# refresh-bio/DSRC

Measured on AMD Instinct MI355X. Metric: raw FASTQ MB/s compressed (bit-identical .dsrc) at -d3 -q2, higher is better.
Workload: dtype u8/u16/u32 integer

## Files before the change

### dsrc_amd/csrc/dsrc_gpu.hip

```cpp
#include <hip/hip_runtime.h>

#include <algorithm>
#include <atomic>
#include <cstdarg>
#include <cstdio>
#include <cstdlib>
#include <cstring>
#include <chrono>
#include <condition_variable>
#include <deque>
#include <functional>
#include <dlfcn.h>
#include <mutex>
#ifndef DSRC_REPLAY_WHATIF
#define DSRC_REPLAY_WHATIF 0
#endif
#include <string>
#include <thread>
#include <vector>

#include "../../include/dsrc_gpu.h"
#include "dsrc_types.h"
#include "k_common.h"
#ifndef RCS_WIDE
// ... 729 lines not shown
	HIPCHK(hipMemcpyAsync(d_desc, desc.data(), sizeof(BlkDesc) * B, hipMemcpyHostToDevice, s));
	HIPCHK(hipMemcpyAsync(d_tplan, tplan.data(), sizeof(TagPlan) * B, hipMemcpyHostToDevice, s));
	HIPCHK(hipMemcpyAsync(d_tres, tres.data(), sizeof(TagFieldRes) * tres.size(), hipMemcpyHostToDevice, s));
	hipLaunchKernelGGL(k_tag_hist, dim3(B), dim3(WG), 0, s, d_in, d_desc, d_state, rp, wpool, wpool, d_tplan, d_tres); KCHK();
	hipLaunchKernelGGL(k_tag_trees, dim3((DSRC_MAX_FIELDS * DSRC_MAX_STRF + 63) / 64, B), dim3(64), 0, s, d_state, wpool, d_tplan, d_tres); KCHK();
	hipLaunchKernelGGL(k_tag_emit, dim3(B), dim3(WG), 0, s, d_in, d_desc, d_state, rp, wpool, spool, wpool, wpool, d_tplan, d_tres); KCHK();
	hipLaunchKernelGGL(k_tag_raw, dim3(B), dim3(WG), 0, s, d_in, d_desc, d_state, rp, wpool, wpool, d_tplan); KCHK();

	if (zero_hi > zero_lo) HIPCHK(hipMemsetAsync(h->arena.base + zero_lo, 0, zero_hi - zero_lo, s));
	HIPCHK(hipMemcpyAsync(d_desc, desc.data(), sizeof(BlkDesc) * B, hipMemcpyHostToDevice, s));
	HIPCHK(hipMemcpyAsync(d_qplan, qplan.data(), sizeof(QuaPlan) * B, hipMemcpyHostToDevice, s));
	HIPCHK(hipMemcpyAsync(d_dplan, dplan.data(), sizeof(QuaPlan) * B, hipMemcpyHostToDevice, s));
	if (NJ)
	{
		HIPCHK(hipMemcpyAsync(d_jobs, jobs.data(), sizeof(CtxJob) * NJ, hipMemcpyHostToDevice, s));
		HIPCHK(hipMemcpyAsync(d_chains, chains.data(), sizeof(RcChain) * NJ, hipMemcpyHostToDevice, s));
	}

	u32 maxq = 1, maxd = 1, max_len = 1, max_qn = 1;
	for (u32 b = 0; b < B; ++b) { maxq = std::max(maxq, st[b].q_total); maxd = std::max(maxd, st[b].d_total); max_len = std::max(max_len, st[b].max_len); max_qn = std::max(max_qn, st[b].q_count); }

	if (qo == 0)
	{
		hipLaunchKernelGGL(k_qpos_hist, dim3(B), dim3(WG), 0, s, d_desc, d_state, rp, d_q, wpool, d_qplan); KCHK();
		hipLaunchKernelGGL(k_qpos_trees, dim3((max_len + 63) / 64, B), dim3(64), 0, s, d_state, wpool, d_qplan); KCHK();
		hipLaunchKernelGGL(k_qpos_emit, dim3(B), dim3(WG), 0, s, d_desc, d_state, rp, d_q, wpool, wpool, d_qplan); KCHK();
		hipLaunchKernelGGL(k_qrle_runs, dim3(B), dim3(WG), 0, s, d_desc, d_state, d_q, wpool, d_qplan); KCHK();
		hipLaunchKernelGGL(k_qrle_hist, dim3(B), dim3(WG), 0, s, d_desc, d_state, d_q, wpool, d_qplan); KCHK();
		hipLaunchKernelGGL(k_qrle_trees, dim3((2 * max_qn + 63) / 64, B), dim3(64), 0, s, d_state, wpool, d_qplan); KCHK();
		hipLaunchKernelGGL(k_qrle_emit, dim3(B), dim3(WG), 0, s, d_desc, d_state, d_q, wpool, wpool, d_qplan); KCHK();
	}
	if (dna_order == 0)
	{
		const u32 gx = std::max(1u, std::min(64u, (maxd / 4 + WG - 1) / WG));
		hipLaunchKernelGGL(k_dna_b2, dim3(gx, B), dim3(WG), 0, s, d_desc, d_state, d_d, wpool); KCHK();
		hipLaunchKernelGGL(k_dna_huff, dim3(B), dim3(WG), 0, s, d_desc, d_state, d_d, wpool, wpool, d_dplan); KCHK();
	}
	hipLaunchKernelGGL(k_dna_none, dim3((B + 63) / 64), dim3(64), 0, s, d_desc, d_state, wpool, B); KCHK();
	h->rc_launches = 0;
	std::function<int(const BkGroup&)> launch_fallback;
	u32* d_bk = use_bk ? AP<u32>(h, o_bk) : nullptr;
	u32* d_redo = AP<u32>(h, o_redo);
	const bool rc_one_lane = hook_env("DSRC_GPU_RC_ONE_LANE") != nullptr;
	if (NJ)
	{
		const u32 nq = (u32)qjobs.size(), nd = (u32)djobs.size();
		const bool sort_atomic = h->sort_atomic;
		hipLaunchKernelGGL(k_rc_headers, dim3((NJ + 63) / 64), dim3(64), 0, s, d_jobs, NJ, d_state, wpool); KCHK();
		HIPCHK(hipMemsetAsync(d_redo, 0, ((size_t)NJ + 2) * 4, s));
		u16* d_bcnt = use_bk ? AP<u16>(h, o_bcnt) : nullptr;
		if (use_bk) HIPCHK(hipMemsetAsync(d_bk, 0, bk_zero_words * 4, s));
		const u32 max_parts = 2048u;
		launch_fallback = [&, sort_atomic, max_parts](const BkGroup& g) -> int
		{
			const u32 cnt = g.hi - g.lo;
			const u32* fb = d_bk + g.fb;
			if (sort_atomic) hipLaunchKernelGGL((k_sort<0, true>), dim3(std::min(cnt, 16u)), dim3(SORT_WG), 0, s, d_jobs, lpool, d_d, d_q, d_qp, d_state, fb);
			else hipLaunchKernelGGL((k_sort<0, false>), dim3(std::min(cnt, 16u)), dim3(SORT_WG), 0, s, d_jobs, lpool, d_d, d_q, d_qp, d_state, fb);
			u32 mxn = 1; for (u32 i = g.lo; i < g.hi; ++i) mxn = std::max(mxn, jobs[i].n);
			const u32 parts = std::max(1u, std::min(max_parts, mxn / 1024u));
			const dim3 rgrid(parts * std::min(cnt, 4u));
#define BK_REPLAY(NN) { hipLaunchKernelGGL(k_replay_seams<NN>, rgrid, dim3(REPLAY_WG), 0, s, d_jobs, const_cast<u64*>(lpool), parts, cnt, fb); \
					hipLaunchKernelGGL((k_replay<NN, 0>), rgrid, dim3(REPLAY_WG), 0, s, d_jobs, lpool, AP<RcPack>(h, 0), parts, cnt, fb); }
			switch (jobs[g.lo].n_alpha)
			{
			case 4: BK_REPLAY(4) break; case 8: BK_REPLAY(8) break; case 16: BK_REPLAY(16) break;
			case 32: BK_REPLAY(32) break; case 64: BK_REPLAY(64) break; default: BK_REPLAY(128) break;
			}
#undef BK_REPLAY
			KCHK();
			return 0;
		};
		for (size_t sl = 0; sl + 1 < slice_lo.size(); ++sl)
		{
			const u32 s_lo = slice_lo[sl], s_hi = slice_lo[sl + 1];
			stage_mark(0);
			if (use_bk)
			{
				u32 slice_bins = 0;
				for (u32 i = s_lo; i < s_hi; ++i) if (jobs[i].bk_on) slice_bins = std::max(slice_bins, (jobs[i].n + BK_BIN - 1) >> BK_TB);
				hipLaunchKernelGGL(k_part, dim3(std::max(1u, slice_bins), s_hi - s_lo), dim3(PART_WG), 0, s, d_jobs + s_lo, lpool, d_d, d_q, d_qp, d_state, d_bk, d_bcnt);
				KCHK();
				stage_mark(0); stage_mark(1);
				if (slice_bins) { hipLaunchKernelGGL(k_binoff, dim3(slice_bins, s_hi - s_lo), dim3(256), 0, s, d_jobs + s_lo, d_bcnt, d_bk); KCHK(); }
				for (const BkGroup& g : bk_groups[sl])
				{
					u32 hb = 0; bool any = false;
					for (u32 i = g.lo; i < g.hi; ++i) if (jobs[i].bk_on) { any = true; hb = std::max(hb, jobs[i].bk_hb); }
					if (!any) continue;
					u32 lbm = 0; for (u32 i = g.lo; i < g.hi; ++i) if (jobs[i].bk_on) lbm = std::max(lbm, jobs[i].bk_lb);
#define BK_LAUNCH(NN, MB, RB) hipLaunchKernelGGL((k_model<NN, MB, RB>), dim3(((1u << hb) + MD_WAVES_FOR(RB) - 1) / MD_WAVES_FOR(RB), g.hi - g.lo), dim3(64 * MD_WAVES_FOR(RB)), 0, s, d_jobs + g.lo, lpool, AP<RcPack>(h, 0), d_bk, d_bcnt, (RcPack*)(d_bk + ((bk_zero_words + 1) & ~(size_t)1)))
#define BK_FINISH(NN) { if ((1u << lbm) * 4 * MdRow<NN>::STRIDE <= 4096) BK_LAUNCH(NN, 0, 4096); \
						else if ((1u << lbm) * 4 * MdRow<NN>::STRIDE <= MD_ROW_BYTES) BK_LAUNCH(NN, 0, MD_ROW_BYTES); \
						else if (lbm <= 10) BK_LAUNCH(NN, 10, MD_ROW_BYTES); \
						else BK_LAUNCH(NN, BK_MAX_LB, MD_ROW_BYTES); }
					switch (jobs[g.lo].n_alpha)
					{
					case 4: BK_FINISH(4) break; case 8: BK_FINISH(8) break; case 16: BK_FINISH(16) break;
					case 32: BK_FINISH(32) break; case 64: BK_FINISH(64) break; default: BK_FINISH(128) break;
					}
#undef BK_LAUNCH
#undef BK_FINISH
					KCHK();
				}
				if (bk_binned && slice_bins) { hipLaunchKernelGGL(k_place, dim3(slice_bins, s_hi - s_lo), dim3(PLACE_WG), 0, s, d_jobs + s_lo, lpool, AP<RcPack>(h, 0), d_bk); KCHK(); }
				for (const BkGroup& g : bk_groups[sl])
				{
					bool known = false;
					for (u32 i = g.lo; i < g.hi; ++i) known = known || !jobs[i].bk_on;
					if (known) { const int rc = launch_fallback(g); if (rc) return rc; }
				}
				stage_mark(1);
				continue;
			}
#ifdef DSRC_SORT_PROBE
			{
				static int shots = 0;
				if (sl == 0 && shots < 2)
				{
					++shots;
					hipEvent_t e0, e1; hipEventCreate(&e0); hipEventCreate(&e1);
#define PROBE_RUN(M) { hipEventRecord(e0, s); if (sort_atomic) hipLaunchKernelGGL((k_sort<M, true>), dim3(s_hi - s_lo), dim3(SORT_WG), 0, s, d_jobs + s_lo, lpool, d_d, d_q, d_qp, d_state, nullptr); else hipLaunchKernelGGL((k_sort<M, false>), dim3(s_hi - s_lo), dim3(SORT_WG), 0, s, d_jobs + s_lo, lpool, d_d, d_q, d_qp, d_state, nullptr); \
					hipEventRecord(e1, s); hipEventSynchronize(e1); float ms = 0; hipEventElapsedTime(&ms, e0, e1); fprintf(stderr, "[probe] k_sort<%u> %u streams: %.2f ms\n", (unsigned)M, s_hi - s_lo, ms); }
					PROBE_RUN(0) PROBE_RUN(0) PROBE_RUN(128) PROBE_RUN(129) PROBE_RUN(130) PROBE_RUN(132) PROBE_RUN(134) PROBE_RUN(136) PROBE_RUN(144) PROBE_RUN(160) PROBE_RUN(192) PROBE_RUN(255)
					hipEventDestroy(e0); hipEventDestroy(e1);
				}
			}
#endif
			if (sort_atomic) hipLaunchKernelGGL((k_sort<0, true>), dim3(s_hi - s_lo), dim3(SORT_WG), 0, s, d_jobs + s_lo, lpool, d_d, d_q, d_qp, d_state, nullptr);
			else hipLaunchKernelGGL((k_sort<0, false>), dim3(s_hi - s_lo), dim3(SORT_WG), 0, s, d_jobs + s_lo, lpool, d_d, d_q, d_qp, d_state, nullptr);
			KCHK();
			stage_mark(0); stage_mark(1);
			for (u32 lo = s_lo; lo < s_hi;)
			{
				u32 hi = lo;
				while (hi < s_hi && jobs[hi].n_alpha == jobs[lo].n_alpha) ++hi;
				const u32 cnt = hi - lo;
				u32 mxn = 1; for (u32 i = lo; i < hi; ++i) mxn = std::max(mxn, jobs[i].n);
				const u32 parts = std::max(1u, std::min(max_parts, mxn / 1024u));
				const dim3 rgrid(parts * cnt);
#ifdef DSRC_SORT_PROBE
				{
					static int shots = 0;
					if ((jobs[lo].n_alpha == 32 || jobs[lo].n_alpha == 4) && lo == s_lo && shots < 4 && (sl == 0 || sl + 2 == slice_lo.size()))
					{
						++shots;
						hipEvent_t e0, e1; hipEventCreate(&e0); hipEventCreate(&e1);
#define RPROBE_RUN(NN, M) { hipEventRecord(e0, s); hipLaunchKernelGGL((k_replay<NN, M>), rgrid, dim3(REPLAY_WG), 0, s, d_jobs + lo, lpool, AP<RcPack>(h, 0), parts, cnt, nullptr); \
						hipEventRecord(e1, s); hipEventSynchronize(e1); float ms = 0; hipEventElapsedTime(&ms, e0, e1); fprintf(stderr, "[probe] k_replay<%d,%d> %u streams x %u parts: %.2f ms\n", NN, M, cnt, parts, ms); }
						hipLaunchKernelGGL(k_replay_seams<32>, rgrid, dim3(REPLAY_WG), 0, s, d_jobs + lo, const_cast<u64*>(lpool), parts, cnt, nullptr);
						if (jobs[lo].n_alpha == 32) { RPROBE_RUN(32, 0) RPROBE_RUN(32, 0) RPROBE_RUN(32, 1) RPROBE_RUN(32, 2) RPROBE_RUN(32, 8) RPROBE_RUN(32, 16) }
						else { RPROBE_RUN(4, 0) RPROBE_RUN(4, 0) RPROBE_RUN(4, 1) RPROBE_RUN(4, 2) RPROBE_RUN(4, 8) RPROBE_RUN(4, 16) }
						hipEventDestroy(e0); hipEventDestroy(e1);
					}
				}
#endif
				switch (jobs[lo].n_alpha)
				{
				case 4:   hipLaunchKernelGGL(k_replay_seams<4>, rgrid, dim3(REPLAY_WG), 0, s, d_jobs + lo, const_cast<u64*>(lpool), parts, cnt, nullptr); hipLaunchKernelGGL((k_replay<4, DSRC_REPLAY_WHATIF>), rgrid, dim3(REPLAY_WG), 0, s, d_jobs + lo, lpool, AP<RcPack>(h, 0), parts, cnt, nullptr); break;
				case 8:   hipLaunchKernelGGL(k_replay_seams<8>, rgrid, dim3(REPLAY_WG), 0, s, d_jobs + lo, const_cast<u64*>(lpool), parts, cnt, nullptr); hipLaunchKernelGGL((k_replay<8, DSRC_REPLAY_WHATIF>), rgrid, dim3(REPLAY_WG), 0, s, d_jobs + lo, lpool, AP<RcPack>(h, 0), parts, cnt, nullptr); break;
				case 16:  hipLaunchKernelGGL(k_replay_seams<16>, rgrid, dim3(REPLAY_WG), 0, s, d_jobs + lo, const_cast<u64*>(lpool), parts, cnt, nullptr); hipLaunchKernelGGL((k_replay<16, DSRC_REPLAY_WHATIF>), rgrid, dim3(REPLAY_WG), 0, s, d_jobs + lo, lpool, AP<RcPack>(h, 0), parts, cnt, nullptr); break;
				case 32:  hipLaunchKernelGGL(k_replay_seams<32>, rgrid, dim3(REPLAY_WG), 0, s, d_jobs + lo, const_cast<u64*>(lpool), parts, cnt, nullptr); hipLaunchKernelGGL((k_replay<32, DSRC_REPLAY_WHATIF>), rgrid, dim3(REPLAY_WG), 0, s, d_jobs + lo, lpool, AP<RcPack>(h, 0), parts, cnt, nullptr); break;
				case 64:  hipLaunchKernelGGL(k_replay_seams<64>, rgrid, dim3(REPLAY_WG), 0, s, d_jobs + lo, const_cast<u64*>(lpool), parts, cnt, nullptr); hipLaunchKernelGGL((k_replay<64, DSRC_REPLAY_WHATIF>), rgrid, dim3(REPLAY_WG), 0, s, d_jobs + lo, lpool, AP<RcPack>(h, 0), parts, cnt, nullptr); break;
				default:  hipLaunchKernelGGL(k_replay_seams<128>, rgrid, dim3(REPLAY_WG), 0, s, d_jobs + lo, const_cast<u64*>(lpool), parts, cnt, nullptr); hipLaunchKernelGGL((k_replay<128, DSRC_REPLAY_WHATIF>), rgrid, dim3(REPLAY_WG), 0, s, d_jobs + lo, lpool, AP<RcPack>(h, 0), parts, cnt, nullptr); break;
				}
				KCHK();
				lo = hi;
			}
			stage_mark(1);
		}
		HIPCHK(hipEventRecord(h->ev[4], s));
		HIPCHK(hipStreamWaitEvent(h->rc_stream, h->ev[4], 0));
		HIPCHK(hipEventRecord(h->ev[2], h->rc_stream));
		if (rc_one_lane) hipLaunchKernelGGL(k_rc, dim3((NJ + RC_LANES - 1) / RC_LANES), dim3(64 * RC_WG_WAVES), 0, h->rc_stream, d_chains, NJ, (const u32*)nullptr, AP<RcPack>(h, 0), wpool, d_state);
		else if (NJ > (u32)hook_int("DSRC_GPU_RC_WIDE_FROM", 640)) hipLaunchKernelGGL(k_rcs<RCS_WIDE>, dim3((NJ + RCS_WIDE - 1) / RCS_WIDE), dim3(64 * RCS_WG_WAVES), 0, h->rc_stream, d_chains, NJ, AP<RcPack>(h, 0), wpool, d_state, (const u32*)d_bk, d_redo);
		else hipLaunchKernelGGL(k_rcs<16>, dim3((NJ + 15) / 16), dim3(64 * RCS_WG_WAVES), 0, h->rc_stream, d_chains, NJ, AP<RcPack>(h, 0), wpool, d_state, (const u32*)d_bk, d_redo);
		KCHK();
		HIPCHK(hipEventRecord(h->ev[3], h->rc_stream));
		HIPCHK(hipEventSynchronize(h->ev[3]));
		h->rc_launches = 1;
	}

	hipLaunchKernelGGL(k_meta_plan, dim3((B + 63) / 64), dim3(64), 0, s, d_state, prm); KCHK();

// ... 1426 lines not shown
```

### dsrc_amd/csrc/k_bucket.h

```cpp
#pragma once
#include <type_traits>
#include "k_rc.h"

#define BK_MAX_HB 10
#define BK_MAX_LB 11
#define BK_LIMIT 524288
#define BK_BIG 16384
#ifndef BK_TB
#define BK_TB 13
#endif
#define BK_BIN (1u << BK_TB)
static_assert(BK_TB == RC6_TB, "a time bin is the unit of k_rc's record layout (rc6_chunk_off)");
#ifndef BK_MAX_BINS
#define BK_MAX_BINS 512
#endif
#define BK_MAX_BINS_WIDE 65536
#define BK_HASH_MUL 0x9E3779B1u


__device__ __forceinline__ u64 bk_rekey(const CtxJob& j, u64 el)
{
	const u32 key = ((u32)(el >> ELEM_CTX_SHIFT) * j.bk_mul) & j.bk_kmask;
	return (el & ((1ull << ELEM_CTX_SHIFT) - 1ull)) | ((u64)key << ELEM_CTX_SHIFT);
}
// ... 81 lines not shown
	constexpr u32 tile_elems = PART_WG * PART_ITEMS;
	const CtxJob j = jobs[blockIdx.y];
	if (!j.bk_on) { if (blockIdx.x == 0 && threadIdx.x == 0) bk_fallback(j, bk); return; }
	const u32 tile = blockIdx.x * tile_elems;
	if (tile >= j.n) return;
	const u32 n = j.n, bins = 1u << j.bk_hb, lb = j.bk_lb;
	const u32 wv = wave_id(), lane = lane_id();
	const u8* sym_src = (j.is_dna ? d_stream : q_stream) + j.src_off;
	const u8* qp = qp_stream + j.src_off;

	for (u32 i = threadIdx.x; i < 256; i += blockDim.x) s_rank[i] = (!j.is_dna && j.translate) ? st[j.blk].q_sym[i] : (u8)i;
	for (u32 i = threadIdx.x; i < PART_WAVES * SORT_MAX_BINS / 2; i += blockDim.x) ((u32*)&s_cnt[0][0])[i] = 0;
	__syncthreads();

	u32 ks[PART_ITEMS], rk[PART_ITEMS];
	const u32 wbase = tile + wv * 64 * PART_ITEMS;
	bool bad = false;
	if (bk_fast8(j) && tile > 0 && tile + tile_elems + 8 <= n)
	{
		static_assert(PART_ITEMS % 8 == 0, "eight consecutive symbols per lane and round");
		static_assert(PART_WAVES * 512 <= BK_BIN / PART_PASSES, "a strip of 512 elements per wave");
		u32* strip = s_tile + wv * 512;
		BkWin w = bk_load8(j, sym_src, wbase + 8 * lane);
#pragma unroll
		for (u32 h = 0; h < PART_ITEMS / 8; ++h)
		{
			u64 e8[8];
			const u32 t0 = wbase + 512 * h + 8 * lane;
			const BkWin wc = w;
			if (h + 1 < PART_ITEMS / 8) w = bk_load8(j, sym_src, t0 + 512);
			if (j.is_dna) bk_elems8_dna(j, wc, t0, e8, &bad); else bk_elems8_qua(j, wc, qp, s_rank, t0, e8);
			if (h) wave_fence();
#pragma unroll
			for (u32 k = 0; k < 8; ++k) strip[8 * lane + k] = bk_keysym(e8[k]);
			wave_fence();
#pragma unroll
			for (u32 k = 0; k < 8; ++k) ks[8 * h + k] = strip[64 * k + lane];
		}
	}
	else
	{
#pragma unroll
		for (u32 k = 0; k < PART_ITEMS; ++k)
		{
			const u32 i = wbase + k * 64 + lane;
			ks[k] = 0;
			if (i < n)
			{
				const u64 e = bk_rekey(j, j.is_dna ? ctx_elem_dna(j, sym_src, i, &bad) : ctx_elem_qua(j, sym_src, qp, s_rank, i));
				ks[k] = bk_keysym(e);
			}
		}
	}
	if (bad) atomicOr(&st[j.blk].err, (u32)DSRC_ERR_REF_UB);
	const u32 shift = 7 + lb;
#pragma unroll
	for (u32 k = 0; k < PART_ITEMS; ++k)
	{
		const u32 i = wbase + k * 64 + lane;
		const u32 d = ks[k] >> shift;
		const u32 sh = (d & 1u) * 16u;
		u32 old = 0;
		if (i < n) old = atomicAdd(&((u32*)s_cnt[wv])[d >> 1], 1u << sh);
		rk[k] = (old >> sh) & 0xFFFFu;
#ifdef DSRC_EMU_BUILD
		(void)__ballot(true);
#endif
	}
	__syncthreads();
	for (u32 d0 = 0, carry = 0; d0 < bins; d0 += PART_WG)
	{
		const u32 dd = d0 + threadIdx.x;
		u32 c[PART_WAVES], tot = 0;
#pragma unroll
		for (u32 w = 0; w < PART_WAVES; ++w) { c[w] = dd < bins ? s_cnt[w][dd] : 0u; tot += c[w]; }
		const u32 inc = wave_incl_scan_dpp(tot);
		if (lane == 63) s_ws[wv] = inc;
		__syncthreads();
		u32 run = carry + inc - tot;
		const u32 nws = (bins - d0 + 63) / 64 < PART_WAVES ? (bins - d0 + 63) / 64 : PART_WAVES;
		for (u32 i = 0; i < nws; ++i) { const u32 x = s_ws[i]; run += i < wv ? x : 0u; carry += x; }
		if (dd < bins)
		{
			bcnt[(u64)j.bk_cnt + (u64)blockIdx.x * bins + dd] = (u16)tot;
#pragma unroll
			for (u32 w = 0; w < PART_WAVES; ++w) { s_cnt[w][dd] = (u16)run; run += c[w]; }
		}
		if (d0 + PART_WG < bins) __syncthreads();
	}
	__syncthreads();
	const u32 lbmask = (1u << lb) - 1u;
	u32* dst = (u32*)(pool + j.elems) + tile;
	const u32 tile_n = n - tile < tile_elems ? n - tile : tile_elems;
	constexpr u32 PIECE = BK_BIN / PART_PASSES;
#pragma unroll
	for (u32 k = 0; k < PART_ITEMS; ++k) rk[k] += (u32)s_cnt[wv][ks[k] >> shift];
#pragma unroll
	for (u32 p = 0; p < PART_PASSES; ++p)
	{
#pragma unroll
		for (u32 k = 0; k < PART_ITEMS; ++k)
		{
			const u32 i = wbase + k * 64 + lane;
			const u32 at = rk[k] - p * PIECE;
			if (i < n && at < PIECE)
				s_tile[at] = (((ks[k] >> 7) & lbmask) << BK_EL_KEY_SHIFT) | ((ks[k] & 0x7Fu) << BK_EL_SYM_SHIFT) | (i & (BK_BIN - 1u));
		}
		__syncthreads();
		if (tile_n == tile_elems)
		{
#pragma unroll
			for (u32 k = 0; k < PIECE / 2 / PART_WG; ++k) ((u64*)(dst + p * PIECE))[k * PART_WG + threadIdx.x] = ((const u64*)s_tile)[k * PART_WG + threadIdx.x];
		}
		else for (u32 q = threadIdx.x; q < PIECE && p * PIECE + q < tile_n; q += PART_WG) dst[p * PIECE + q] = s_tile[q];
		if (p + 1 < PART_PASSES) __syncthreads();
	}
}

#define MD_WAVES_FOR(ROW_BYTES) ((ROW_BYTES) <= 4096 ? 4 : 2)
#define MD_ROW_BYTES 8192
#define MD_NONE 0xFFFFFFFFu

template <int N> struct MdRow
{
	static constexpr int B = N <= 4 ? 2 : N <= 8 ? 3 : N <= 16 ? 4 : N <= 32 ? 5 : N <= 64 ? 6 : 7;
	static constexpr int L4 = B / 2;
	static constexpr bool R2 = (B & 1) != 0;
	static constexpr u32 W64 = ((1u << (2 * L4)) - 1u) / 3u;
	static constexpr u32 STRIDE = 2 * W64 + (R2 ? N / 2 : 0);
};

template <int N> __device__ __forceinline__ u32 md_init_word(u32 x)
{
	typedef MdRow<N> G;
	if (x >= 2 * G::W64) return 0x00010001u;
	const u32 w = x >> 1;
	const u32 l = w >= 5 ? 2u : w >= 1 ? 1u : 0u;
	const u32 v = (u32)N >> (2 * (l + 1));
	return v | (v << 16);
}

template <int N> __device__ __forceinline__ u32 md_total(const u32* row)
{
	const u64 v = *(const unsigned long long*)row;
	return ((u32)v & 0xFFFFu) + ((u32)v >> 16) + ((u32)(v >> 32) & 0xFFFFu) + (u32)(v >> 48);
}

template <int N> __device__ __forceinline__ void md_rescale(u32* row)
{
	typedef MdRow<N> G;
	unsigned long long* r64 = (unsigned long long*)row;
	if (G::R2)
		for (u32 x = 0; x < (u32)N / 2; ++x)
		{
			const u32 v = row[2 * G::W64 + x];
			u32 a = v & 0xFFFFu, b = v >> 16;
			a -= a >> 1; b -= b >> 1;
			row[2 * G::W64 + x] = a | (b << 16);
		}
	for (int l = G::L4 - 1; l >= 0; --l)
	{
		const u32 base = ((1u << (2 * l)) - 1u) / 3u, nw = 1u << (2 * l);
		for (u32 w = 0; w < nw; ++w)
		{
			u64 v = 0;
			if (!G::R2 && l == G::L4 - 1)
			{
				const u64 o = r64[base + w];
#pragma unroll
				for (u32 q = 0; q < 4; ++q) { u32 x = (u32)(o >> (16 * q)) & 0xFFFFu; x -= x >> 1; v |= (u64)x << (16 * q); }
			}
			else
			{
#pragma unroll
				for (u32 q = 0; q < 4; ++q)
				{
					const u32 c = 4 * w + q;
					u32 sum;
					if (l == G::L4 - 1) { const u32 p = row[2 * G::W64 + c]; sum = (p & 0xFFFFu) + (p >> 16); }
					else { const u64 o = r64[((1u << (2 * (l + 1))) - 1u) / 3u + c]; sum = ((u32)o & 0xFFFFu) + ((u32)o >> 16) + ((u32)(o >> 32) & 0xFFFFu) + (u32)(o >> 48); }
					v |= (u64)sum << (16 * q);
				}
			}
			r64[base + w] = v;
		}
	}
}

template <int N> __device__ __forceinline__ u64 md_code(u32* row, u32 sym)
{
	typedef MdRow<N> G;
	unsigned long long* r64 = (unsigned long long*)row;
	u32 cum = 0, tot = 0, f = 0;
#pragma unroll
	for (int l = 0; l < G::L4; ++l)
	{
		const u32 q = (sym >> (G::B - 2 * l - 2)) & 3u;
		const u32 wi = ((1u << (2 * l)) - 1u) / 3u + (l ? sym >> (G::B - 2 * l) : 0u);
		const u64 old = atomicAdd(&r64[wi], 2ull << (16 * q));
		const u64 below = old & ((1ull << (16 * q)) - 1ull);
		cum += ((u32)below & 0xFFFFu) + ((u32)below >> 16) + ((u32)(below >> 32) & 0xFFFFu);
		if (l == 0) tot = ((u32)old & 0xFFFFu) + ((u32)old >> 16) + ((u32)(old >> 32) & 0xFFFFu) + (u32)(old >> 48);
		f = (u32)(old >> (16 * q)) & 0xFFFFu;
	}
	if (G::R2)
	{
		const u32 old = atomicAdd(&row[2 * G::W64 + (sym >> 1)], (sym & 1u) ? (2u << 16) : 2u);
		cum += (sym & 1u) ? (old & 0xFFFFu) : 0u;
		f = (sym & 1u) ? (old >> 16) : (old & 0xFFFFu);
	}
	return (u64)f | ((u64)cum << 16) | ((u64)tot << 32);
}

__global__ void __launch_bounds__(256) k_binoff(const CtxJob* jobs, u16* bcnt, const u32* bk)
{
	const CtxJob j = jobs[blockIdx.y];
	const u32 bin = blockIdx.x;
	if (!j.bk_on || bk[j.jid] || (bin << BK_TB) >= j.n) return;
	const u32 bins = 1u << j.bk_hb;
	u16* row = bcnt + j.bk_cnt + (u64)bin * bins;
	u32 c[4], mine = 0;
#pragma unroll
	for (u32 k = 0; k < 4; ++k)
	{
		const u32 b = 4 * threadIdx.x + k;
		c[k] = b < bins ? (u32)row[b] : 0u;
		mine += c[k];
	}
	u32 tot;
	u32 run = block_excl_scan(mine, &tot);
#pragma unroll
	for (u32 k = 0; k < 4; ++k)
	{
		const u32 b = 4 * threadIdx.x + k;
		if (b < bins) row[b] = (u16)run;
		run += c[k];
	}
}

template <bool SMALL> struct MdMapT { typedef u8 T; static constexpr u32 NONE = 0xFFu, CLAIM = 0x80u; };
template <> struct MdMapT<false> { typedef u16 T; static constexpr u32 NONE = 0xFFFFu, CLAIM = 0x8000u; };

#ifndef MD_AHEAD
#define MD_AHEAD 3
#endif
#ifndef MD_ROTATE_ALL
#define MD_ROTATE_ALL 0
#endif
template <int N, int MAPBITS, int ROW_BYTES>
__global__ void __launch_bounds__(64 * MD_WAVES_FOR(ROW_BYTES)) k_model(const CtxJob* jobs, const u64* pool, RcPack* rec_pool, u32* bk, const u16* bcnt, RcPack* nowhere)
{
	constexpr u32 STRIDE = MdRow<N>::STRIDE;
	constexpr u32 ROWS = ROW_BYTES / (4 * STRIDE);
	constexpr u32 MD_WAVES = MD_WAVES_FOR(ROW_BYTES);
	typedef MdMapT<(ROWS <= 127)> Map;
	typedef typename Map::T map_t;
	__shared__ map_t s_map[MD_WAVES][1 << MAPBITS];
	__shared__ unsigned long long s_rows[MD_WAVES][ROW_BYTES / 8];
	__shared__ u16 s_off[MD_WAVES][BK_MAX_BINS];
	__shared__ u16 s_num[MD_WAVES][BK_MAX_BINS];
	__shared__ u8 s_head[MD_WAVES][64];
	constexpr u32 limit = (1u << 16) - 2u * N;
	const CtxJob j = jobs[blockIdx.y];
	const u32 w = wave_id(), lane = lane_id();
#ifndef MD_XCD_MAP
#define MD_XCD_MAP 1
#endif
	u32 bx = blockIdx.x;
	if (MD_XCD_MAP && gridDim.x % 8u == 0) bx = (((bx & 7u) + blockIdx.y) & 7u) * (gridDim.x >> 3) + (bx >> 3);
	const u32 bucket = bx * MD_WAVES + w;
	const u32 buckets = 1u << j.bk_hb;
	if (!j.bk_on || bucket >= buckets || bk[j.jid]) return;
	const u32* src = (const u32*)(pool + j.elems);
	RcPack* recs = j.bk_binned ? (RcPack*)pool + j.elems_b : rec_pool + j.trip;
	const u32 keys = 1u << j.bk_lb;
	const bool binned = j.bk_binned != 0;
	map_t* map = s_map[w]; u32* rows = (u32*)s_rows[w]; u16* off = s_off[w]; u16* num = s_num[w]; u8* head = s_head[w];
	const u32 n_bins = (j.n + BK_BIN - 1) >> BK_TB;

	const bool wide = n_bins > j.bk_narrow_bins;
	auto tile_info = [&](u32 b, u32* o_out) -> u32
	{
		const u16* row = bcnt + (u64)j.bk_cnt + (u64)b * buckets;
		const u32 o = row[bucket];
		const u32 tile_n = j.n - (b << BK_TB) < BK_BIN ? j.n - (b << BK_TB) : BK_BIN;
		*o_out = o;
		return (bucket + 1 < buckets ? (u32)row[bucket + 1] : tile_n) - o;
	};
	u32 nb = 0;
	for (u32 b = lane; b < n_bins; b += 64)
	{
		u32 o;
		const u32 c = tile_info(b, &o);
		if (!wide) { off[b] = (u16)o; num[b] = (u16)c; }
		nb += c;
	}
	head[lane] = 0xFFu;
	for (u32 d = 32; d >= 1; d >>= 1) nb += __shfl_xor(nb, (int)d);
	if (!nb) return;
	if (nb > j.bk_limit)
	{
		if (lane == 0) bk_fallback(j, bk);
		return;
	}
	const bool may_rescale = (u32)N + 2u * nb + 128u >= (1u << 16) - 2u * N;
	wave_fence();

	u32 g_bin = 0, g_pos = 0, g_tot = 0, left = nb;
	u32 g_inc = 0, g_f = 0, g_off = 0;
	auto load_group = [&]()
	{
		const u32 b = g_bin + lane;
		u32 c = 0;
		if (b < n_bins) { if (wide) c = tile_info(b, &g_off); else c = (u32)num[b]; }
		g_inc = wave_incl_scan_dpp(c); g_f = g_inc - c;
		g_tot = wave_last(g_inc); g_pos = 0;
	};
	load_group();
	const bool big = nb >= j.bk_big;
	auto next_window = [&]() -> u32
	{
		if (!left) return MD_NONE;
		while (g_pos >= g_tot && g_bin < n_bins) { g_bin += 64; load_group(); }
		if (g_pos >= g_tot) { left = 0; return MD_NONE; }
		if (big)
		{
			const u64 in = __ballot(g_f <= g_pos && g_pos < g_inc);
			const u32 k0 = (u32)__ffsll((long long)in) - 1u;
			const u32 e0 = (u32)__builtin_amdgcn_readlane((int)g_inc, (int)k0);
			if (e0 - g_pos >= 64u)
			{
				const u32 f0 = (u32)__builtin_amdgcn_readlane((int)g_f, (int)k0);
				const u32 bin = g_bin + k0;
				const u32 o0 = wide ? (u32)__builtin_amdgcn_readlane((int)g_off, (int)k0) : (u32)off[bin & (BK_MAX_BINS - 1u)];
				const u32 idx = (bin << BK_TB) + o0 + (g_pos - f0) + lane;
				g_pos += 64u; left -= 64u;
				return idx;
			}
		}
		const int rel = (int)(g_f - g_pos);
		if (g_inc > g_f && g_inc > g_pos && rel < 64) head[rel > 0 ? rel : 0] = (u8)lane;
		wave_fence();
		const u32 hd = head[lane];
		wave_fence();
		head[lane] = 0xFFu;
		const u64 hm = __ballot(hd != 0xFFu);
		const u64 le = hm & (lanemask_lt() | (1ull << lane));
		const u32 hl = le ? 63u - (u32)__clzll((long long)le) : 0u;
		const u32 k = (u32)__shfl((int)hd, (int)hl) & 63u;
		const u32 k0 = (u32)__builtin_amdgcn_readfirstlane((int)hd) & 63u;
		const u32 f0 = (u32)__builtin_amdgcn_readlane((int)g_f, (int)k0);
		const u32 r = lane - hl + (hl == 0 ? g_pos - f0 : 0u);
		const u32 avail = g_tot - g_pos < 64 ? g_tot - g_pos : 64u;
		const u32 bin = g_bin + k;
		const u32 ok = wide ? (u32)__shfl((int)g_off, (int)k) : (u32)off[bin & (BK_MAX_BINS - 1u)];
		const u32 idx = lane < avail ? (bin << BK_TB) + ok + r : MD_NONE;
		g_pos += avail; left -= avail;
		return idx;
	};

	u32 elq[MD_AHEAD], ixq[MD_AHEAD];
#pragma unroll
	for (u32 k = 0; k < MD_AHEAD; ++k) { ixq[k] = next_window(); elq[k] = src[ixq[k] != MD_NONE ? ixq[k] : 0u]; }
	if (MAPBITS) for (u32 i = lane; i < keys; i += 64) map[i] = (map_t)Map::NONE;
	for (u32 i = lane; i < (MAPBITS ? ROWS : keys) * STRIDE; i += 64) rows[i] = md_init_word<N>(i % STRIDE);
	wave_fence();

	u32 n_rows = 0;
#ifdef MD_PROFILE
	u64 pf[6] = {0, 0, 0, 0, 0, 0}; u32 pf_n = 0;
#define MD_T(k, dep) { u64 t_; asm volatile("s_memtime %0\n s_waitcnt lgkmcnt(0)" : "=s"(t_) : "s"(dep) : "memory"); pf[k] += t_ - pf_t; pf_t = t_; }
#else
#define MD_T(k, dep)
#endif
	auto walk = [&](auto resc_tag)
	{
	constexpr bool RESC = decltype(resc_tag)::value;
	u32 coded = 0, dry = 0;
	auto step = [&](u32& el_slot, u32& ix_slot) -> bool
	{
#ifdef MD_PROFILE
		u64 pf_t; asm volatile("s_memtime %0\n s_waitcnt lgkmcnt(0)" : "=s"(pf_t) :: "memory"); ++pf_n;
#endif
		const u32 el = el_slot, ix = ix_slot;
		const bool valid = ix != MD_NONE;
		const u32 n_valid = (u32)__popcll(__ballot(valid));
		coded += n_valid;
		dry = (n_valid || left) ? 0u : dry + 1u;
		const u32 ix_new = next_window();
		const u32 el_new = src[ix_new != MD_NONE ? ix_new : 0u];
		MD_T(0, __builtin_amdgcn_readfirstlane((int)ix_new))
		MD_T(1, __builtin_amdgcn_readfirstlane((int)el))

		const u32 key = el >> BK_EL_KEY_SHIFT, sym = (el >> BK_EL_SYM_SHIFT) & (u32)(N - 1);
		u32 rid = key;
		if (MAPBITS)
		{
			rid = valid ? (u32)map[key] : 0u;
			const bool need = valid && rid == Map::NONE;
			if (__ballot(need))
			{
				if (need) map[key] = (map_t)(Map::CLAIM | lane);
				wave_fence();
				const bool leader = need && (u32)map[key] == (Map::CLAIM | lane);
				const u64 lm = __ballot(leader);
				const u32 mine = n_rows + (u32)__popcll(lm & lanemask_lt());
				n_rows += (u32)__popcll(lm);
				if (n_rows > ROWS)
				{
					if (lane == 0) bk_fallback(j, bk);
					return false;
				}
				wave_fence();
				if (leader) map[key] = (map_t)mine;
				wave_fence();
				if (need) rid = (u32)map[key];
			}
		}
		MD_T(2, __builtin_amdgcn_readfirstlane((int)rid))
		u64 rec = 0;
		u32* row = rows + rid * STRIDE;
		const bool near = RESC && valid && md_total<N>(row) + 128u >= limit;
		if (RESC && __ballot(near))
		{
			const u64 vm = __ballot(valid);
			for (u32 l = 0; l < 64 && ((vm >> l) & 1ull); ++l)
			{
				if (lane == l)
				{
					if (md_total<N>(row) >= limit) md_rescale<N>(row);
					rec = md_code<N>(row, sym);
				}
				wave_fence();
			}
		}
		else if (valid) rec = md_code<N>(row, sym);
#ifdef DSRC_EMU_BUILD
		(void)__ballot(true);
#endif
		MD_T(3, __builtin_amdgcn_readfirstlane((int)(u32)rec))
		if (binned)
		{
			RcPack* to = recs + ix;
			if (!valid) to = nowhere + lane;
			*to = rec | ((u64)(el & (BK_BIN - 1u)) << 48);
		}
		else
		{
			const u32 t = (ix & ~(BK_BIN - 1u)) | (el & (BK_BIN - 1u));
			u8* chunk = (u8*)recs + rc6_chunk_off(t >> 6);
			u32* p32 = valid ? (u32*)chunk + (t & 63u) : (u32*)(nowhere + lane);
			u16* p16 = valid ? (u16*)(chunk + 256) + (t & 63u) : (u16*)(nowhere + lane) + 2;
			*p32 = (u32)rec; *p16 = (u16)(rec >> 32);
		}
		el_slot = el_new; ix_slot = ix_new;
		MD_T(4, 0)
		return coded < nb && dry <= MD_AHEAD;
	};
	if (MD_ROTATE_ALL || MAPBITS != 0)
		for (bool go = nb != 0; go;)
		{
#pragma unroll
			for (u32 k = 0; k < MD_AHEAD; ++k) if (go) go = step(elq[k], ixq[k]);
		}
	else
		for (bool go = nb != 0; go;)
		{
			u32 e = elq[0], i = ixq[0];
			go = step(e, i);
#pragma unroll
			for (u32 k = 0; k + 1 < MD_AHEAD; ++k) { elq[k] = elq[k + 1]; ixq[k] = ixq[k + 1]; }
			elq[MD_AHEAD - 1] = e; ixq[MD_AHEAD - 1] = i;
		}
	};
	if (may_rescale) walk(std::true_type()); else walk(std::false_type());
#ifdef MD_PROFILE
	if (lane == 0 && nb >= 65536u && (bucket & 3u) == 0)
		printf("MD N=%d nb=%u rows=%u windows=%u cycles/window: book %u wait %u map %u code %u store %u\n", N, nb, n_rows, pf_n,
			(u32)(pf[0] / pf_n), (u32)(pf[1] / pf_n), (u32)(pf[2] / pf_n), (u32)(pf[3] / pf_n), (u32)(pf[4] / pf_n));
#endif
}

#ifndef PLACE_WG
#define PLACE_WG 512
#endif
#ifndef PLACE_PASSES
#define PLACE_PASSES 2
#endif
__global__ void __launch_bounds__(PLACE_WG) k_place(const CtxJob* jobs, const u64* pool, RcPack* rec_pool, const u32* bk)
{
	constexpr u32 PER = BK_BIN / PLACE_WG, HALF = BK_BIN / PLACE_PASSES;
	__shared__ u64 s_rec[HALF];
	const CtxJob j = jobs[blockIdx.y];
	if (!j.bk_on || !j.bk_binned || bk[j.jid]) return;
	const u32 bin = blockIdx.x;
	const u32 t0 = bin << BK_TB;
	if (t0 >= j.n) return;
	const u32 cnt = j.n - t0 < BK_BIN ? j.n - t0 : BK_BIN;
	const RcPack* r = (const RcPack*)pool + j.elems_b + t0;
	u8* out = (u8*)(rec_pool + j.trip) + (size_t)(t0 >> 6) * RC6_CHUNK_BYTES;
	u64 v[PER];
#pragma unroll
	for (u32 k = 0; k < PER; ++k) v[k] = threadIdx.x + k * PLACE_WG < cnt ? r[threadIdx.x + k * PLACE_WG] : ~0ull;
#pragma unroll
	for (u32 p = 0; p < PLACE_PASSES; ++p)
	{
		const u32 lo = p * HALF;
#pragma unroll
		for (u32 k = 0; k < PER; ++k)
		{
			const u32 t = (u32)(v[k] >> 48) - lo;
			if (t < HALF) s_rec[t] = v[k] & 0xFFFFFFFFFFFFull;
		}
		__syncthreads();
		for (u32 i = threadIdx.x; i < HALF && lo + i < cnt; i += PLACE_WG)
		{
			const u32 t = lo + i;
			const u64 v6 = s_rec[i];
			u8* c = out + (t >> 6) * RC6_CHUNK_BYTES;
			((u32*)c)[t & 63u] = (u32)v6;
			((u16*)(c + 256))[t & 63u] = (u16)(v6 >> 32);
		}
		if (p + 1 < PLACE_PASSES) __syncthreads();
	}
}
```

Before: 65510.

## Fold bin-offset scan into k_part and specialize k_model on binned layout

k_part now writes exclusive per-bin offsets directly, so the separate k_binoff scan kernel and its launch are removed. k_model gains a compile-time BINNED template parameter, reads bin offsets from registers instead of LDS, and makes several values wave-uniform. It also uses clamped element loads, a rotating prefetch ring with a spare slot, and a fast store path when all 64 lanes are valid. The host always launches the binned variant unless test hooks are enabled. There is a risk if the unbinned layout is still needed at runtime or if the written offsets differ in meaning from what k_binoff produced.

```diff
diff --git a/dsrc_amd/csrc/dsrc_gpu.hip b/dsrc_amd/csrc/dsrc_gpu.hip
--- a/dsrc_amd/csrc/dsrc_gpu.hip
+++ b/dsrc_amd/csrc/dsrc_gpu.hip
@@ -835,14 +835,18 @@
 				hipLaunchKernelGGL(k_part, dim3(std::max(1u, slice_bins), s_hi - s_lo), dim3(PART_WG), 0, s, d_jobs + s_lo, lpool, d_d, d_q, d_qp, d_state, d_bk, d_bcnt);
 				KCHK();
 				stage_mark(0); stage_mark(1);
-				if (slice_bins) { hipLaunchKernelGGL(k_binoff, dim3(slice_bins, s_hi - s_lo), dim3(256), 0, s, d_jobs + s_lo, d_bcnt, d_bk); KCHK(); }
 				for (const BkGroup& g : bk_groups[sl])
 				{
 					u32 hb = 0; bool any = false;
 					for (u32 i = g.lo; i < g.hi; ++i) if (jobs[i].bk_on) { any = true; hb = std::max(hb, jobs[i].bk_hb); }
 					if (!any) continue;
 					u32 lbm = 0; for (u32 i = g.lo; i < g.hi; ++i) if (jobs[i].bk_on) lbm = std::max(lbm, jobs[i].bk_lb);
-#define BK_LAUNCH(NN, MB, RB) hipLaunchKernelGGL((k_model<NN, MB, RB>), dim3(((1u << hb) + MD_WAVES_FOR(RB) - 1) / MD_WAVES_FOR(RB), g.hi - g.lo), dim3(64 * MD_WAVES_FOR(RB)), 0, s, d_jobs + g.lo, lpool, AP<RcPack>(h, 0), d_bk, d_bcnt, (RcPack*)(d_bk + ((bk_zero_words + 1) & ~(size_t)1)))
+#ifdef DSRC_GPU_TEST_HOOKS
+#define BK_LAUNCH(NN, MB, RB) do { if (bk_binned) BK_LAUNCH_B(NN, MB, RB, true); else BK_LAUNCH_B(NN, MB, RB, false); } while (0)
+#else
+#define BK_LAUNCH(NN, MB, RB) BK_LAUNCH_B(NN, MB, RB, true)
+#endif
+#define BK_LAUNCH_B(NN, MB, RB, BN) hipLaunchKernelGGL((k_model<NN, MB, RB, BN>), dim3(((1u << hb) + MD_WAVES_FOR(RB) - 1) / MD_WAVES_FOR(RB), g.hi - g.lo), dim3(64 * MD_WAVES_FOR(RB)), 0, s, d_jobs + g.lo, lpool, AP<RcPack>(h, 0), d_bk, d_bcnt, (RcPack*)(d_bk + ((bk_zero_words + 1) & ~(size_t)1)))
 #define BK_FINISH(NN) { if ((1u << lbm) * 4 * MdRow<NN>::STRIDE <= 4096) BK_LAUNCH(NN, 0, 4096); \
 						else if ((1u << lbm) * 4 * MdRow<NN>::STRIDE <= MD_ROW_BYTES) BK_LAUNCH(NN, 0, MD_ROW_BYTES); \
 						else if (lbm <= 10) BK_LAUNCH(NN, 10, MD_ROW_BYTES); \
@@ -853,6 +857,7 @@
 					case 32: BK_FINISH(32) break; case 64: BK_FINISH(64) break; default: BK_FINISH(128) break;
 					}
 #undef BK_LAUNCH
+#undef BK_LAUNCH_B
 #undef BK_FINISH
 					KCHK();
 				}
diff --git a/dsrc_amd/csrc/k_bucket.h b/dsrc_amd/csrc/k_bucket.h
--- a/dsrc_amd/csrc/k_bucket.h
+++ b/dsrc_amd/csrc/k_bucket.h
@@ -187,7 +187,7 @@
 		for (u32 i = 0; i < nws; ++i) { const u32 x = s_ws[i]; run += i < wv ? x : 0u; carry += x; }
 		if (dd < bins)
 		{
-			bcnt[(u64)j.bk_cnt + (u64)blockIdx.x * bins + dd] = (u16)tot;
+			bcnt[(u64)j.bk_cnt + (u64)blockIdx.x * bins + dd] = (u16)run;
 #pragma unroll
 			for (u32 w = 0; w < PART_WAVES; ++w) { s_cnt[w][dd] = (u16)run; run += c[w]; }
 		}
@@ -317,32 +317,6 @@
 	return (u64)f | ((u64)cum << 16) | ((u64)tot << 32);
 }
 
-__global__ void __launch_bounds__(256) k_binoff(const CtxJob* jobs, u16* bcnt, const u32* bk)
-{
-	const CtxJob j = jobs[blockIdx.y];
-	const u32 bin = blockIdx.x;
-	if (!j.bk_on || bk[j.jid] || (bin << BK_TB) >= j.n) return;
-	const u32 bins = 1u << j.bk_hb;
-	u16* row = bcnt + j.bk_cnt + (u64)bin * bins;
-	u32 c[4], mine = 0;
-#pragma unroll
-	for (u32 k = 0; k < 4; ++k)
-	{
-		const u32 b = 4 * threadIdx.x + k;
-		c[k] = b < bins ? (u32)row[b] : 0u;
-		mine += c[k];
-	}
-	u32 tot;
-	u32 run = block_excl_scan(mine, &tot);
-#pragma unroll
-	for (u32 k = 0; k < 4; ++k)
-	{
-		const u32 b = 4 * threadIdx.x + k;
-		if (b < bins) row[b] = (u16)run;
-		run += c[k];
-	}
-}
-
 template <bool SMALL> struct MdMapT { typedef u8 T; static constexpr u32 NONE = 0xFFu, CLAIM = 0x80u; };
 template <> struct MdMapT<false> { typedef u16 T; static constexpr u32 NONE = 0xFFFFu, CLAIM = 0x8000u; };
 
@@ -352,7 +326,13 @@
 #ifndef MD_ROTATE_ALL
 #define MD_ROTATE_ALL 0
 #endif
-template <int N, int MAPBITS, int ROW_BYTES>
+#ifndef MD_SPARE
+#define MD_SPARE 1
+#endif
+#define MD_SLOTS (MD_AHEAD + MD_SPARE)
+__device__ __forceinline__ u32 wave_uniform(u32 v) { return (u32)__builtin_amdgcn_readfirstlane((int)v); }
+
+template <int N, int MAPBITS, int ROW_BYTES, bool BINNED>
 __global__ void __launch_bounds__(64 * MD_WAVES_FOR(ROW_BYTES)) k_model(const CtxJob* jobs, const u64* pool, RcPack* rec_pool, u32* bk, const u16* bcnt, RcPack* nowhere)
 {
 	constexpr u32 STRIDE = MdRow<N>::STRIDE;
@@ -367,7 +347,7 @@
 	__shared__ u8 s_head[MD_WAVES][64];
 	constexpr u32 limit = (1u << 16) - 2u * N;
 	const CtxJob j = jobs[blockIdx.y];
-	const u32 w = wave_id(), lane = lane_id();
+	const u32 w = wave_uniform(wave_id()), lane = lane_id();
 #ifndef MD_XCD_MAP
 #define MD_XCD_MAP 1
 #endif
@@ -375,11 +355,13 @@
 	if (MD_XCD_MAP && gridDim.x % 8u == 0) bx = (((bx & 7u) + blockIdx.y) & 7u) * (gridDim.x >> 3) + (bx >> 3);
 	const u32 bucket = bx * MD_WAVES + w;
 	const u32 buckets = 1u << j.bk_hb;
-	if (!j.bk_on || bucket >= buckets || bk[j.jid]) return;
-	const u32* src = (const u32*)(pool + j.elems);
-	RcPack* recs = j.bk_binned ? (RcPack*)pool + j.elems_b : rec_pool + j.trip;
+	if (!j.bk_on || bucket >= buckets) return;
+	if (wave_uniform(bk[j.jid])) return;
+	const u8* src = (const u8*)(pool + j.elems);
+	const u32 last = j.n - 1u;
+	auto load_el = [&](u32 ix) -> u32 { return *(const u32*)(src + (size_t)(u32)((ix < last ? ix : last) << 2)); };
+	u8* recs = BINNED ? (u8*)((RcPack*)pool + j.elems_b) : (u8*)(rec_pool + j.trip);
 	const u32 keys = 1u << j.bk_lb;
-	const bool binned = j.bk_binned != 0;
 	map_t* map = s_map[w]; u32* rows = (u32*)s_rows[w]; u16* off = s_off[w]; u16* num = s_num[w]; u8* head = s_head[w];
 	const u32 n_bins = (j.n + BK_BIN - 1) >> BK_TB;
 
@@ -402,6 +384,7 @@
 	}
 	head[lane] = 0xFFu;
 	for (u32 d = 32; d >= 1; d >>= 1) nb += __shfl_xor(nb, (int)d);
+	nb = wave_uniform(nb);
 	if (!nb) return;
 	if (nb > j.bk_limit)
 	{
@@ -417,9 +400,9 @@
 	{
 		const u32 b = g_bin + lane;
 		u32 c = 0;
-		if (b < n_bins) { if (wide) c = tile_info(b, &g_off); else c = (u32)num[b]; }
+		if (b < n_bins) { if (wide) c = tile_info(b, &g_off); else { c = (u32)num[b]; g_off = (u32)off[b]; } }
 		g_inc = wave_incl_scan_dpp(c); g_f = g_inc - c;
-		g_tot = wave_last(g_inc); g_pos = 0;
+		g_tot = wave_uniform(wave_last(g_inc)); g_pos = 0;
 	};
 	load_group();
 	const bool big = nb >= j.bk_big;
@@ -436,9 +419,8 @@
 			if (e0 - g_pos >= 64u)
 			{
 				const u32 f0 = (u32)__builtin_amdgcn_readlane((int)g_f, (int)k0);
-				const u32 bin = g_bin + k0;
-				const u32 o0 = wide ? (u32)__builtin_amdgcn_readlane((int)g_off, (int)k0) : (u32)off[bin & (BK_MAX_BINS - 1u)];
-				const u32 idx = (bin << BK_TB) + o0 + (g_pos - f0) + lane;
+				const u32 o0 = (u32)__builtin_amdgcn_readlane((int)g_off, (int)k0);
+				const u32 idx = ((g_bin + k0) << BK_TB) + o0 + (g_pos - f0) + lane;
 				g_pos += 64u; left -= 64u;
 				return idx;
 			}
@@ -458,15 +440,15 @@
 		const u32 r = lane - hl + (hl == 0 ? g_pos - f0 : 0u);
 		const u32 avail = g_tot - g_pos < 64 ? g_tot - g_pos : 64u;
 		const u32 bin = g_bin + k;
-		const u32 ok = wide ? (u32)__shfl((int)g_off, (int)k) : (u32)off[bin & (BK_MAX_BINS - 1u)];
+		const u32 ok = (u32)__shfl((int)g_off, (int)k);
 		const u32 idx = lane < avail ? (bin << BK_TB) + ok + r : MD_NONE;
 		g_pos += avail; left -= avail;
 		return idx;
 	};
 
-	u32 elq[MD_AHEAD], ixq[MD_AHEAD];
-#pragma unroll
-	for (u32 k = 0; k < MD_AHEAD; ++k) { ixq[k] = next_window(); elq[k] = src[ixq[k] != MD_NONE ? ixq[k] : 0u]; }
+	u32 elq[MD_SLOTS], ixq[MD_SLOTS];
+#pragma unroll
+	for (u32 k = 0; k < MD_AHEAD; ++k) { ixq[k] = next_window(); elq[k] = load_el(ixq[k]); }
 	if (MAPBITS) for (u32 i = lane; i < keys; i += 64) map[i] = (map_t)Map::NONE;
 	for (u32 i = lane; i < (MAPBITS ? ROWS : keys) * STRIDE; i += 64) rows[i] = md_init_word<N>(i % STRIDE);
 	wave_fence();
@@ -482,18 +464,17 @@
 	{
 	constexpr bool RESC = decltype(resc_tag)::value;
 	u32 coded = 0, dry = 0;
-	auto step = [&](u32& el_slot, u32& ix_slot) -> bool
+	auto step = [&](const u32 el, const u32 ix, u32& el_next, u32& ix_next) -> bool
 	{
 #ifdef MD_PROFILE
 		u64 pf_t; asm volatile("s_memtime %0\n s_waitcnt lgkmcnt(0)" : "=s"(pf_t) :: "memory"); ++pf_n;
 #endif
-		const u32 el = el_slot, ix = ix_slot;
 		const bool valid = ix != MD_NONE;
 		const u32 n_valid = (u32)__popcll(__ballot(valid));
 		coded += n_valid;
 		dry = (n_valid || left) ? 0u : dry + 1u;
-		const u32 ix_new = next_window();
-		const u32 el_new = src[ix_new != MD_NONE ? ix_new : 0u];
+		const u32 ix_new = ix_next = next_window();
+		el_next = load_el(ix_new);
 		MD_T(0, __builtin_amdgcn_readfirstlane((int)ix_new))
 		MD_T(1, __builtin_amdgcn_readfirstlane((int)el))
 
@@ -544,35 +525,43 @@
 		(void)__ballot(true);
 #endif
 		MD_T(3, __builtin_amdgcn_readfirstlane((int)(u32)rec))
-		if (binned)
-		{
-			RcPack* to = recs + ix;
-			if (!valid) to = nowhere + lane;
-			*to = rec | ((u64)(el & (BK_BIN - 1u)) << 48);
+		if (BINNED)
+		{
+			const u64 out = rec | ((u64)(el & (BK_BIN - 1u)) << 48);
+			if (n_valid == 64u) *(RcPack*)(recs + (size_t)(u32)(ix << 3)) = out;
+			else
+			{
+				RcPack* to = (RcPack*)recs + ix;
+				if (!valid) to = nowhere + lane;
+				*to = out;
+			}
 		}
 		else
 		{
 			const u32 t = (ix & ~(BK_BIN - 1u)) | (el & (BK_BIN - 1u));
-			u8* chunk = (u8*)recs + rc6_chunk_off(t >> 6);
-			u32* p32 = valid ? (u32*)chunk + (t & 63u) : (u32*)(nowhere + lane);
-			u16* p16 = valid ? (u16*)(chunk + 256) + (t & 63u) : (u16*)(nowhere + lane) + 2;
-			*p32 = (u32)rec; *p16 = (u16)(rec >> 32);
-		}
-		el_slot = el_new; ix_slot = ix_new;
+			const u32 at = rc6_chunk_off(t >> 6) + 4u * (t & 63u), at16 = rc6_chunk_off(t >> 6) + 256u + 2u * (t & 63u);
+			if (n_valid == 64u) { *(u32*)(recs + (size_t)at) = (u32)rec; *(u16*)(recs + (size_t)at16) = (u16)(rec >> 32); }
+			else
+			{
+				u32* p32 = valid ? (u32*)(recs + (size_t)at) : (u32*)(nowhere + lane);
+				u16* p16 = valid ? (u16*)(recs + (size_t)at16) : (u16*)(nowhere + lane) + 2;
+				*p32 = (u32)rec; *p16 = (u16)(rec >> 32);
+			}
+		}
 		MD_T(4, 0)
 		return coded < nb && dry <= MD_AHEAD;
 	};
 	if (MD_ROTATE_ALL || MAPBITS != 0)
-		for (bool go = nb != 0; go;)
-		{
-#pragma unroll
-			for (u32 k = 0; k < MD_AHEAD; ++k) if (go) go = step(elq[k], ixq[k]);
+		for (;;)
+		{
+#pragma unroll
+			for (u32 k = 0; k < MD_SLOTS; ++k) if (!step(elq[k], ixq[k], elq[(k + MD_AHEAD) % MD_SLOTS], ixq[(k + MD_AHEAD) % MD_SLOTS])) return;
 		}
 	else
 		for (bool go = nb != 0; go;)
 		{
-			u32 e = elq[0], i = ixq[0];
-			go = step(e, i);
+			u32 e, i;
+			go = step(elq[0], ixq[0], e, i);
 #pragma unroll
 			for (u32 k = 0; k + 1 < MD_AHEAD; ++k) { elq[k] = elq[k + 1]; ixq[k] = ixq[k + 1]; }
 			elq[MD_AHEAD - 1] = e; ixq[MD_AHEAD - 1] = i;
```

Result: faster. 67100, median of 6 (+2.4%).
